# TxCorpi0x/concrete

Measured on AMD Instinct MI355X. Metric: PBS/sec (whole node) at N=1024 batch=4096; achieved HBM GB/s, higher is better.
Workload: dtype u64

## Files before the change

### concrete_amd/csrc/pbs.hip

```cpp
#include <type_traits>

#include "common.hpp"
#include "fft512.hpp"
#include "kernel_util.hpp"
#include "pbs.hpp"
#include "pbs1024_plan.hpp"
#include "pbs_hex.hpp"
#include "pbs_launch.hpp"

namespace chip {

static_assert(MAGIC_ALL_3 == RND_MAGIC_BITS + (RND_MAGIC_BITS << 22) + (RND_MAGIC_BITS << 43),
              "three limbs at shifts 0, 22, 43");

#ifndef FWD_LAST_VIA_WINDOW
#define FWD_LAST_VIA_WINDOW 1
#endif
#ifndef FWD_TW2_EARLY
#define FWD_TW2_EARLY 1
#endif
#ifndef DIAG_NOMAC
#define DIAG_NOMAC 0
#endif

#ifndef FWD_XBATCH
#define FWD_XBATCH 2
#endif
#ifndef PAIR_FLAGS
#define PAIR_FLAGS 1
#endif

#if defined(DIAG_NOXBAR)
constexpr bool XBAR = false;
#else
constexpr bool XBAR = true;
#endif
__device__ __forceinline__ void pair_signal(uint32_t* f, int h, uint32_t& cnt) {
  if constexpr (XBAR) group_signal<2>(f, h, cnt);
}
__device__ __forceinline__ void pair_wait(uint32_t* f, int h, uint32_t cnt, const SyncGuard& guard) {
  if constexpr (XBAR) group_wait<2>(f, h, cnt, guard);
}
__device__ __forceinline__ void xchg_barrier(uint32_t* f, int h, uint32_t& cnt, const SyncGuard& guard) {
  if constexpr (!XBAR) asm volatile("s_waitcnt lgkmcnt(0)" ::: "memory");
  else if constexpr (PAIR_FLAGS) group_sync<2>(f, h, cnt, guard);
  else pair_barrier();
}

template <int P, int L, bool RESID, bool STAMPS>
__global__ void __launch_bounds__(P * 128, 2)
pbs1024_pair_kernel(uint64_t* __restrict__ out, const uint64_t* __restrict__ out_idx,
                    const uint64_t* __restrict__ luts, const uint64_t* __restrict__ lut_idx,
                    const uint64_t* __restrict__ in, const uint64_t* __restrict__ in_idx,
                    const cplx* __restrict__ fbsk, uint32_t n, uint32_t base_log, uint32_t num_samples,
                    unsigned long long* __restrict__ resid_out, SyncGuard guard) {
  constexpr int K = 1, K1 = 2, N = 1024, LOG2_2N = 11, LIMBS = 3, RQ = K1 * L;
  constexpr int PER_I = K1 * LIMBS * RQ * 512;
  static_assert(XCH_SLOTS <= (int)PBS1024_XCH_SLOTS, "transpose scratch");
  static_assert(FFT512_TABLE_ENTRIES * sizeof(cplx) == PBS1024_TABLE_BYTES, "table bytes");
  constexpr int NW = 2 * P;
  constexpr int GROUP = L * 512;
  constexpr int NGRP = K1 * K1 * LIMBS;
  constexpr int GLDS = GROUP / 64 / NW;
  static_assert(GROUP % (64 * NW) == 0, "group split");

  extern __shared__ __attribute__((aligned(16))) char smem[];
  cplx* tbl = reinterpret_cast<cplx*>(smem);
  cplx* xch_all = tbl + FFT512_TABLE_ENTRIES;
  cplx* ring = xch_all + NW * PBS1024_XCH_SLOTS;
  uint32_t* pflags = reinterpret_cast<uint32_t*>(ring + 3 * GROUP);

  const int w = __builtin_amdgcn_readfirstlane(threadIdx.x >> 6);
  const int h = w & 1;
  uint32_t* pf = pflags + (w - h);
  const uint64_t hsign = (uint64_t)h << 63;
  const int lane = threadIdx.x & 63;
  const uint32_t s = blockIdx.x * P + (w >> 1);
  const bool active = s < num_samples;
  cplx* xch = xch_all + w * PBS1024_XCH_SLOTS;
  uint64_t* xch64 = reinterpret_cast<uint64_t*>(xch);
  cplx* mybox = xch;
  const cplx* partnerbox = xch_all + (w ^ 1) * PBS1024_XCH_SLOTS;
  cplx* partnermail = xch_all + (w ^ 1) * PBS1024_XCH_SLOTS;

  static_assert(NGRP % 3 == 0, "ring slot of a group must not depend on the step");
  const cplx* key_w = fbsk + (uint64_t)w * GLDS * 64;
  cplx* ring_w = ring + w * GLDS * 64;
  const uint32_t lane_b = (uint32_t)lane * (uint32_t)sizeof(cplx);
  auto issue_group = [&](const cplx* key_step, int r) __attribute__((always_inline)) {
    ring_issue<GLDS, true>(reinterpret_cast<const char*>(key_step + r * GROUP), ring_w + (r % 3) * GROUP, lane_b);
  };
  if (n > 0) {
    issue_group(key_w, 0);
    issue_group(key_w, 1);
  }

  build_fft512_tables(tbl, threadIdx.x, P * 128);
  if (lane == 0) pflags[w] = 0u;
  uint32_t pcnt = 0;
  __syncthreads();
  const Fft512Tables T = fft512_tables_at(tbl);

  const uint64_t* lwe = in + (active ? (in_idx ? in_idx[s] : s) : 0) * (uint64_t)(n + 1);
  const uint64_t* lut = luts + (active && lut_idx ? lut_idx[s] : 0ull) * (uint64_t)(K1 * N);

  uint64_t B[16];
  {
    const uint32_t bt = active ? modswitch(lwe[n], LOG2_2N) : 0u;
#pragma unroll
    for (int m = 0; m < 16; ++m) {
      const uint32_t src = (uint32_t)(lane + 64 * m + bt) & (2 * N - 1);
      const uint64_t v = active ? lut[h * N + (src & (N - 1))] : 0ull;
      B[m] = src < N ? 0ull - v : v;
    }
  }

  const int nrep = 64 - L * (int)base_log;
  const int logB = (int)base_log;
  const int32_t neg_base = -(1 << logB);
  const uint32_t half_m1 = (1u << (logB - 1)) - 1u;
  double max_resid = 0.0;
  uint64_t acc_t[NSTAMP] = {};
  uint64_t t_begin = 0, tp = 0;
  if constexpr (STAMPS) t_begin = stamp();

  cplx tw3[4];
  fwd_p3_tw(tw3, T, lane);

  uint64_t a_next = active ? lwe[0] : 0ull;
  for (uint32_t i = 0; i < n; ++i) {
    const cplx* key_step = key_w + (uint64_t)i * PER_I;
    const uint64_t ai = a_next;
    if (i + 1 < n) a_next = active ? lwe[i + 1] : 0ull;

    const uint32_t at = modswitch(ai, LOG2_2N);
    if constexpr (STAMPS) {
      tp = stamp();
      acc_t[7] += ai != 0ull && at != 0u;
    }

    uint32_t st[16];
    {
#pragma unroll
      for (int m = 0; m < 16; ++m) xch64[lane + 64 * m] = B[m];
      wave_lds_fence();
      const uint32_t o0 = ((uint32_t)(lane - (int)at) << 3) + 8u * N;
      const uint32_t khi = 1u << (nrep - 33);
      uint64_t rv[16];
#pragma unroll
      for (int m = 0; m < 16; ++m)
        rv[m] = *reinterpret_cast<const uint64_t*>(reinterpret_cast<const char*>(xch64) + ((o0 + 512u * m) & 8191u));
      __builtin_amdgcn_sched_barrier(0);
#pragma unroll
      for (int m = 0; m < 16; ++m) {
        const uint32_t o = o0 + 512u * m;
        const uint32_t s32 = (uint32_t)((int32_t)(o << 18) >> 31);
        const uint64_t rvs = rv[m] ^ (((uint64_t)s32 << 32) | s32);
        const uint64_t x = B[m] + rvs + (uint64_t)(s32 & 1u);
        st[m] = ((uint32_t)(x >> 32) + khi) >> (nrep - 32);
      }
      wave_lds_fence();
    }
    if constexpr (STAMPS) {
      uint64_t t = stamp();
      acc_t[0] += t - tp;
      tp = t;
    }

    cplx Xo[L][4], Xp[L][4];
    constexpr int XB = FWD_XBATCH;
#pragma unroll
    for (int q0 = 0; q0 < L; q0 += XB) {
      const int nq = (q0 + XB <= L) ? XB : L - q0;
      cplx out[XB][4];
      {
#pragma unroll
        for (int t = 0; t < XB; ++t) {
          if (t < nq) {
            cplx v[8];
            int32_t d[16];
#pragma unroll
            for (int m = 0; m < 16; ++m)
              d[m] = decomp_level32(st[m], (uint32_t)((q0 + t) * logB), logB, half_m1, neg_base, q0 + t + 1 < L);
#pragma unroll
            for (int m = 0; m < 8; ++m) v[m] = {(double)d[m], (double)d[m + 8]};
            cplx tw2[4];
            fwd_p2_tw(tw2, T, lane >> 3);
            if (FWD_TW2_EARLY) __builtin_amdgcn_sched_barrier(0);
            fft512_fwd_tw(v, xch, lane, tw2, tw3, hsign, [&]() __attribute__((always_inline)) {
              if (q0 > 0 && t == 0) pair_wait(pf, h, pcnt, guard);
            });
#pragma unroll
            for (int j = 0; j < 4; ++j) {
              Xo[q0 + t][j] = v[j];
              out[t][j] = v[4 + j];
            }
          }
        }
#pragma unroll
        for (int t = 0; t < XB; ++t)
          if (t < nq)
#pragma unroll
            for (int j = 0; j < 4; ++j) mybox[(t * 4 + j) * 64 + lane] = out[t][j];
      }
      const bool last_batch = q0 + XB >= L;
      if (!last_batch || !FWD_LAST_VIA_WINDOW) {
        xchg_barrier(pf, h, pcnt, guard);
#pragma unroll
        for (int t = 0; t < XB; ++t)
          if (t < nq)
#pragma unroll
            for (int j = 0; j < 4; ++j) Xp[q0 + t][j] = partnerbox[(t * 4 + j) * 64 + lane];
      }
#pragma unroll
      for (int t = 0; t < XB; ++t)
        if (t < nq)
#pragma unroll
          for (int j = 0; j < 4; ++j) pin(Xo[q0 + t][j]);
      if (q0 + XB < L) pair_signal(pf, h, pcnt);
    }
    if constexpr (STAMPS) {
      uint64_t t = stamp();
      acc_t[1] += t - tp;
      tp = t;
    }

    auto recombine = [&](const cplx (&v)[8], auto LIc) __attribute__((always_inline)) {
      constexpr int lr = decltype(LIc)::value;
#pragma unroll
      for (int m = 0; m < 8; ++m) {
        const double tr = RND_MAGIC - v[m].re, ti = RND_MAGIC - v[m].im;
        if constexpr (RESID) {
          max_resid = fmax(max_resid, fabs(v[m].re - (RND_MAGIC - tr)));
          max_resid = fmax(max_resid, fabs(v[m].im - (RND_MAGIC - ti)));
        }
        if constexpr (lr == 0) {
          B[m] += (uint64_t)__double_as_longlong(tr) - MAGIC_ALL_3;
          B[m + 8] += (uint64_t)__double_as_longlong(ti) - MAGIC_ALL_3;
        } else {
          B[m] += (uint64_t)__double_as_longlong(tr) << limb_shift(lr);
          B[m + 8] += (uint64_t)__double_as_longlong(ti) << limb_shift(lr);
        }
      }
    };
    static_for<0, LIMBS>([&](auto LI) __attribute__((always_inline)) {
      constexpr int li = decltype(LI)::value;
      cplx Ymine[4];
#pragma unroll
      for (int co = 0; co < K1; ++co) {
        cplx Y[4];
        if constexpr (DIAG_NOMAC) {
#pragma unroll
          for (int j = 0; j < 4; ++j) Y[j] = {0.0, 0.0};
        }
#pragma unroll
        for (int ro = 0; ro < K1; ++ro) {
          const int r = (li * K1 + co) * K1 + ro;
          const bool last_step = i + 1 >= n;
          if constexpr (STAMPS) {
            uint64_t t = stamp();
            acc_t[2] += t - tp;
            tp = t;
          }
          if (r + 1 < NGRP || !last_step) wait_vmcnt<GLDS>();
          else wait_vmcnt<0>();
          if constexpr (STAMPS) {
            uint64_t t = stamp();
            acc_t[8] += t - tp;
            tp = t;
          }
#ifndef DIAG_NOBAR
          pair_barrier();
#endif
          if constexpr (STAMPS) {
            uint64_t t = stamp();
            acc_t[5] += t - tp;
            tp = t;
          }
#ifndef DIAG_NODMA
          if (r + 2 < NGRP) issue_group(key_step, r + 2);
          else if (!last_step) issue_group(key_step + PER_I, r + 2 - NGRP);
#endif
          if constexpr (FWD_LAST_VIA_WINDOW && li == 0) {
            if (co == 0 && ro == 0) {
              constexpr int QL = (L - 1) / FWD_XBATCH * FWD_XBATCH;
#pragma unroll
              for (int q = QL; q < L; ++q)
#pragma unroll
                for (int j = 0; j < 4; ++j) Xp[q][j] = partnerbox[((q - QL) * 4 + j) * 64 + lane];
            }
          }
          const cplx* G = ring + (r % 3) * GROUP + (4 * h) * 64 + lane;
          cplx gv[L][4];
#pragma unroll
          for (int q = 0; q < L; ++q)
#pragma unroll
            for (int j = 0; j < 4; ++j) gv[q][j] = G[(q * 8 + j) * 64];
#pragma unroll
          for (int q = 0; q < (DIAG_NOMAC ? 0 : L); ++q) {
#pragma unroll
            for (int j = 0; j < 4; ++j) {
              const cplx x = ro == 0 ? Xo[q][j] : Xp[q][j];
              if (ro == 0 && q == 0) {
                Y[j].re = __builtin_fma(x.re, gv[q][j].re, -x.im * gv[q][j].im);
                Y[j].im = __builtin_fma(x.re, gv[q][j].im, x.im * gv[q][j].re);
              } else {
                Y[j].re = __builtin_fma(x.re, gv[q][j].re, __builtin_fma(-x.im, gv[q][j].im, Y[j].re));
                Y[j].im = __builtin_fma(x.re, gv[q][j].im, __builtin_fma(x.im, gv[q][j].re, Y[j].im));
              }
            }
          }
#pragma unroll
          for (int j = 0; j < 4; ++j) pin(Y[j]);
        }
        if (co == 0) {
#pragma unroll
          for (int j = 0; j < 4; ++j) Ymine[j] = Y[j];
        } else {
#pragma unroll
          for (int j = 0; j < 4; ++j) partnermail[j * 64 + lane] = Y[j];
        }
      }
      if constexpr (STAMPS) {
        uint64_t t = stamp();
        acc_t[2] += t - tp;
        tp = t;
      }
      xchg_barrier(pf, h, pcnt, guard);
      cplx vp[8];
#pragma unroll
      for (int j = 0; j < 4; ++j) {
        vp[j] = Ymine[j];
        vp[4 + j] = mybox[j * 64 + lane];
      }
      if constexpr (STAMPS) {
        uint64_t t = stamp();
        acc_t[3] += t - tp;
        tp = t;
      }
      cplx gi2[4];
      inv_p2_stage_tw(gi2, T, lane & 7);
      fft512_inv_tw(vp, xch, T, lane, gi2, hsign);
      recombine(vp, LI);
#pragma unroll
      for (int m = 0; m < 16; ++m) pin(B[m]);
      if constexpr (RESID) pin(max_resid);
      if constexpr (STAMPS) {
        uint64_t t = stamp();
        acc_t[4] += t - tp;
        tp = t;
      }
    });
  }

  if constexpr (STAMPS) {
    acc_t[6] = stamp() - t_begin;
    if (lane == 0 && resid_out) {
      unsigned long long* dst = resid_out + ((uint64_t)blockIdx.x * NW + w) * NSTAMP;
      for (int q = 0; q < NSTAMP; ++q) dst[q] = acc_t[q];
    }
  }

  uint64_t* o = out + (active ? (out_idx ? out_idx[s] : s) : 0) * (uint64_t)(K * N + 1);
  if (!active) {
  } else if (h == 0) {
#pragma unroll
    for (int m = 0; m < 16; ++m) xch64[lane + 64 * m] = B[m];
    wave_lds_fence();
#pragma unroll
    for (int m = 0; m < 16; ++m) {
      const int j = lane + 64 * m;
      const uint64_t v = xch64[(N - j) & (N - 1)];
      o[j] = j == 0 ? 0ull - v : v;
    }
  } else if (lane == 0) {
    o[K * N] = 0ull - B[0];
  }

  if constexpr (RESID && !STAMPS) report_resid(max_resid, lane, active, resid_out);
}

#ifndef SLOT_PF
#define SLOT_PF 6
#endif
#ifndef SLOT_FWD_PAIR
#define SLOT_FWD_PAIR 1
#endif
#ifndef SLOT_Y_EARLY
#define SLOT_Y_EARLY 1
#endif
#ifndef SLOT_QMAJOR
#define SLOT_QMAJOR 1
#endif
#ifndef SLOT_DEFAULT
#define SLOT_DEFAULT 1
#endif
constexpr int SLOT_MBOX = 512;
constexpr size_t pbs1024_pair_slot_lds_bytes() {
  return PBS1024_TABLE_BYTES + 2 * (size_t)PBS_PAIRS * (PBS1024_XCH_SLOTS + SLOT_MBOX) * 16 + 16;
}

__device__ __forceinline__ void slot_signal(uint32_t* ctr, int lane, uint32_t& cnt) {
  asm volatile("" ::: "memory");
  ++cnt;
  if (lane == 0) __hip_atomic_fetch_add(ctr, 1u, __ATOMIC_RELAXED, __HIP_MEMORY_SCOPE_WORKGROUP);
}

template <bool RESID, bool STAMPS>
__global__ void __launch_bounds__(PBS_PAIRS * 128, 2)
pbs1024_pair_slot_kernel(uint64_t* __restrict__ out, const uint64_t* __restrict__ out_idx,
                         const uint64_t* __restrict__ luts, const uint64_t* __restrict__ lut_idx,
                         const uint64_t* __restrict__ in, const uint64_t* __restrict__ in_idx,
                         const cplx* __restrict__ fbsk, uint32_t n, uint32_t base_log, uint32_t num_samples,
                         unsigned long long* __restrict__ resid_out, SyncGuard guard) {
  constexpr int K = 1, K1 = 2, N = 1024, LOG2_2N = 11, LIMBS = 3, L = 3, P = PBS_PAIRS, NW = 2 * P;
  constexpr int GROUP = L * 512;
  constexpr int PER_I = K1 * K1 * LIMBS * GROUP;
  constexpr int NKEY = LIMBS * K1 * K1 * L;
  constexpr int PF = SLOT_PF;
  constexpr int XS = (int)PBS1024_XCH_SLOTS, MB = SLOT_MBOX;
  static_assert(NW == 8, "one frequency slot per wave");
  static_assert(NKEY % PF == 0, "a key value's register must not depend on the step");
  static_assert(XCH_SLOTS <= XS, "transpose scratch");

  extern __shared__ __attribute__((aligned(16))) char smem[];
  cplx* tbl = reinterpret_cast<cplx*>(smem);
  cplx* xch_all = tbl + FFT512_TABLE_ENTRIES;
  cplx* mbox_all = xch_all + NW * XS;
  uint32_t* ctr = reinterpret_cast<uint32_t*>(mbox_all + NW * MB);

  const int w = __builtin_amdgcn_readfirstlane(threadIdx.x >> 6);
  const int h = w & 1;
  const int lane = threadIdx.x & 63;
  const uint32_t s = blockIdx.x * P + (w >> 1);
  const bool active = s < num_samples;
  cplx* xch = xch_all + w * XS;
  uint64_t* xch64 = reinterpret_cast<uint64_t*>(xch);
  cplx* mybox = mbox_all + w * MB + lane;
  cplx* slotbox = mbox_all + w * 64 + lane;

  const bool flip = w >= 4;
  const cplx* key_w = fbsk + (w * 64 + (flip ? 3 * GROUP : 0));
  const int gstride = flip ? -GROUP : GROUP;
  auto key_load = [&](const cplx* key_step, int t) __attribute__((always_inline)) {
    const int li = t / (K1 * K1 * L), co = t / (K1 * L) % K1, e = t % (K1 * L);
    const int ro = SLOT_QMAJOR ? e % K1 : e / L, q = SLOT_QMAJOR ? e / K1 : e % L, cr = co * K1 + ro;
    return (key_step + (li * K1 * K1 * GROUP + q * 512) + cr * gstride)[lane];
  };
  cplx g[PF] = {};
  if (n > 0) {
#pragma unroll
    for (int t = 0; t < PF; ++t) g[t] = key_load(key_w, t);
  }

  build_fft512_tables(tbl, threadIdx.x, P * 128);
  if (threadIdx.x == 0) *ctr = 0u;
  uint32_t rcnt = 0;
  __syncthreads();
  const Fft512Tables T = fft512_tables_at(tbl);

  const uint64_t* lwe = in + (active ? (in_idx ? in_idx[s] : s) : 0) * (uint64_t)(n + 1);
  const uint64_t* lut = luts + (active && lut_idx ? lut_idx[s] : 0ull) * (uint64_t)(K1 * N);

  uint64_t B[16];
  {
    const uint32_t bt = active ? modswitch(lwe[n], LOG2_2N) : 0u;
#pragma unroll
    for (int m = 0; m < 16; ++m) {
      const uint32_t src = (uint32_t)(lane + 64 * m + bt) & (2 * N - 1);
      const uint64_t v = active ? lut[h * N + (src & (N - 1))] : 0ull;
      B[m] = src < N ? 0ull - v : v;
    }
  }

  const int nrep = 64 - L * (int)base_log;
  const int logB = (int)base_log;
  const int32_t neg_base = -(1 << logB);
  const uint32_t half_m1 = (1u << (logB - 1)) - 1u;
  double max_resid = 0.0;
  uint64_t acc_t[NSTAMP] = {};
  uint64_t t_begin = 0, tp = 0;
  auto lap = [&](int k) __attribute__((always_inline)) {
    if constexpr (STAMPS) {
      const uint64_t t = stamp();
      acc_t[k] += t - tp;
      tp = t;
    }
  };
  if constexpr (STAMPS) t_begin = stamp();

  cplx tw3[4];
  fwd_p3_tw(tw3, T, lane);

  uint64_t a_next = active && n > 0 ? lwe[0] : 0ull;
  for (uint32_t i = 0; i < n; ++i) {
    const cplx* key_step = key_w + (uint64_t)i * PER_I;
    const cplx* key_next = i + 1 < n ? key_step + PER_I : key_step;
    const uint64_t ai = a_next;
    if (i + 1 < n) a_next = active ? lwe[i + 1] : 0ull;
    const uint32_t at = modswitch(ai, LOG2_2N);
    if constexpr (STAMPS) {
      tp = stamp();
      acc_t[7] += ai != 0ull && at != 0u;
    }

    uint32_t st[16];
    {
#pragma unroll
      for (int m = 0; m < 16; ++m) xch64[lane + 64 * m] = B[m];
      wave_lds_fence();
      const uint32_t o0 = ((uint32_t)(lane - (int)at) << 3) + 8u * N;
      const uint32_t khi = 1u << (nrep - 33);
      uint64_t rv[16];
#pragma unroll
      for (int m = 0; m < 16; ++m)
        rv[m] = *reinterpret_cast<const uint64_t*>(reinterpret_cast<const char*>(xch64) + ((o0 + 512u * m) & 8191u));
      __builtin_amdgcn_sched_barrier(0);
#pragma unroll
      for (int m = 0; m < 16; ++m) {
        const uint32_t o = o0 + 512u * m;
        const uint32_t s32 = (uint32_t)((int32_t)(o << 18) >> 31);
        const uint64_t rvs = rv[m] ^ (((uint64_t)s32 << 32) | s32);
        const uint64_t x = B[m] + rvs + (uint64_t)(s32 & 1u);
        st[m] = ((uint32_t)(x >> 32) + khi) >> (nrep - 32);
      }
      wave_lds_fence();
    }
    lap(0);

    cplx X[L][NW];
    cplx hold[8];
    (void)hold;
#pragma unroll
    for (int q = 0; q < L; ++q) {
      cplx v[8];
      int32_t d[16];
#pragma unroll
      for (int m = 0; m < 16; ++m)
        d[m] = decomp_level32(st[m], (uint32_t)(q * logB), logB, half_m1, neg_base, q + 1 < L);
#pragma unroll
      for (int m = 0; m < 8; ++m) v[m] = {(double)d[m], (double)d[m + 8]};
      cplx tw2[4];
      fwd_p2_tw(tw2, T, lane >> 3);
      if (FWD_TW2_EARLY) __builtin_amdgcn_sched_barrier(0);
#if SLOT_FWD_PAIR
      fft512_fwd_tw(v, xch, lane, tw2, tw3, 0ull, [&]() __attribute__((always_inline)) {
        if (q == 2) spin_until_ge(ctr, NW * rcnt, guard);
      });
      if (q == 0) {
#pragma unroll
        for (int k = 0; k < 8; ++k) hold[k] = v[k];
      } else {
#pragma unroll
        for (int k = 0; k < 8; ++k) {
          if (q == 1) mybox[k * 64] = hold[k], xch[k * 64 + lane] = v[k];
          else mybox[k * 64] = v[k];
        }
        lap(1);
        pair_barrier();
        lap(5);
#pragma unroll
        for (int u = 0; u < NW; ++u) {
          if (q == 1) X[0][u] = slotbox[u * MB], X[1][u] = xch_all[u * XS + w * 64 + lane];
          else X[2][u] = slotbox[u * MB];
        }
        slot_signal(ctr, lane, rcnt);
      }
#else
      fft512_fwd_tw(v, xch, lane, tw2, tw3, 0ull, []() __attribute__((always_inline)) {});
      if (q > 0) spin_until_ge(ctr, NW * rcnt, guard);
#pragma unroll
      for (int k = 0; k < 8; ++k) mybox[k * 64] = v[k];
      lap(1);
      pair_barrier();
      lap(5);
#pragma unroll
      for (int u = 0; u < NW; ++u) X[q][u] = slotbox[u * MB];
      slot_signal(ctr, lane, rcnt);
#endif
    }
    lap(1);

    auto recombine = [&](const cplx (&v)[8], auto LIc) __attribute__((always_inline)) {
      constexpr int lr = decltype(LIc)::value;
#pragma unroll
      for (int m = 0; m < 8; ++m) {
        const double tr = RND_MAGIC - v[m].re, ti = RND_MAGIC - v[m].im;
        if constexpr (RESID) {
          max_resid = fmax(max_resid, fabs(v[m].re - (RND_MAGIC - tr)));
          max_resid = fmax(max_resid, fabs(v[m].im - (RND_MAGIC - ti)));
        }
        if constexpr (lr == 0) {
          B[m] += (uint64_t)__double_as_longlong(tr) - MAGIC_ALL_3;
          B[m + 8] += (uint64_t)__double_as_longlong(ti) - MAGIC_ALL_3;
        } else {
          B[m] += (uint64_t)__double_as_longlong(tr) << limb_shift(lr);
          B[m + 8] += (uint64_t)__double_as_longlong(ti) << limb_shift(lr);
        }
      }
    };
    auto window = [&](auto LIc, auto COc) __attribute__((always_inline)) {
      constexpr int li = decltype(LIc)::value, co = decltype(COc)::value;
      cplx Y[P];
#pragma unroll
      for (int e = 0; e < K1 * L; ++e) {
        const int ro = SLOT_QMAJOR ? e % K1 : e / L, q = SLOT_QMAJOR ? e / K1 : e % L;
        const int t = (li * K1 + co) * K1 * L + e;
        const cplx gv = g[t % PF];
#pragma unroll
        for (int c = 0; c < P; ++c) {
          const cplx x = X[q][2 * c + ro];
          if (e == 0) {
            Y[c].re = __builtin_fma(x.re, gv.re, -x.im * gv.im);
            Y[c].im = __builtin_fma(x.re, gv.im, x.im * gv.re);
          } else {
            Y[c].re = __builtin_fma(x.re, gv.re, __builtin_fma(-x.im, gv.im, Y[c].re));
            Y[c].im = __builtin_fma(x.re, gv.im, __builtin_fma(x.im, gv.re, Y[c].im));
          }
        }
        g[t % PF] = t + PF < NKEY ? key_load(key_step, t + PF) : key_load(key_next, t + PF - NKEY);
      }
#pragma unroll
      for (int c = 0; c < P; ++c) pin(Y[c]);
      if (co == 0) spin_until_ge(ctr, NW * rcnt, guard);
#pragma unroll
      for (int c = 0; c < P; ++c) mbox_all[(2 * c + co) * MB + w * 64 + lane] = Y[c];
    };
    if (SLOT_Y_EARLY) window(std::integral_constant<int, 0>{}, std::integral_constant<int, 0>{});
    static_for<0, LIMBS>([&](auto LI) __attribute__((always_inline)) {
      constexpr int li = decltype(LI)::value;
      if (!SLOT_Y_EARLY) window(LI, std::integral_constant<int, 0>{});
      window(LI, std::integral_constant<int, 1>{});
      lap(2);
      pair_barrier();
      lap(5);
      cplx vp[8];
#pragma unroll
      for (int k = 0; k < 8; ++k) vp[k] = mybox[k * 64];
      slot_signal(ctr, lane, rcnt);
      lap(3);
      if constexpr (SLOT_Y_EARLY && li + 1 < LIMBS) {
        window(std::integral_constant<int, li + 1>{}, std::integral_constant<int, 0>{});
        lap(2);
      }
      cplx gi2[4];
      inv_p2_stage_tw(gi2, T, lane & 7);
      fft512_inv_tw(vp, xch, T, lane, gi2, 0ull);
      recombine(vp, LI);
#pragma unroll
      for (int m = 0; m < 16; ++m) pin(B[m]);
      if constexpr (RESID) pin(max_resid);
      lap(4);
    });
  }

  if constexpr (STAMPS) {
    acc_t[6] = stamp() - t_begin;
    if (lane == 0 && resid_out) {
      unsigned long long* dst = resid_out + ((uint64_t)blockIdx.x * NW + w) * NSTAMP;
      for (int q = 0; q < NSTAMP; ++q) dst[q] = acc_t[q];
    }
  }

  uint64_t* o = out + (active ? (out_idx ? out_idx[s] : s) : 0) * (uint64_t)(K * N + 1);
  if (!active) {
  } else if (h == 0) {
#pragma unroll
    for (int m = 0; m < 16; ++m) xch64[lane + 64 * m] = B[m];
    wave_lds_fence();
#pragma unroll
    for (int m = 0; m < 16; ++m) {
      const int j = lane + 64 * m;
      const uint64_t v = xch64[(N - j) & (N - 1)];
      o[j] = j == 0 ? 0ull - v : v;
    }
  } else if (lane == 0) {
    o[K * N] = 0ull - B[0];
  }

  if constexpr (RESID && !STAMPS) report_resid(max_resid, lane, active, resid_out);
}

template <bool RESID, bool STAMPS>
static int launch_slot_t(const PbsArgs& a) {
  constexpr int P = PBS_PAIRS;
  const size_t lds = pbs1024_pair_slot_lds_bytes();
  static_assert(pbs1024_pair_slot_lds_bytes() <= 160 * 1024, "LDS of one CU");
  if (!pbs1024_exact(1, 3, a.base_log)) {
    set_error("pbs: N=1024 l=3 logB=%u is outside the exact range", a.base_log);
    return -2;
  }
  return launch_fused(pbs1024_pair_slot_kernel<RESID, STAMPS>, P, P * 128, lds, a);
}

static int launch_slot(const PbsArgs& a) {
  static const bool stamps = getenv("CONCRETE_HIP_PBS_STAMPS") && atoi(getenv("CONCRETE_HIP_PBS_STAMPS"));
  if (stamps) return launch_slot_t<true, true>(a);
  return a.resid ? launch_slot_t<true, false>(a) : launch_slot_t<false, false>(a);
}

template <int P, int L, bool RESID, bool STAMPS>
static int launch_pair_t(const PbsArgs& a) {
  const size_t lds = pbs1024_pair_lds_bytes(L, P);
  if (!pbs1024_exact(1, L, a.base_log)) {
    set_error("pbs: N=1024 l=%d logB=%u is outside the exact range", L, a.base_log);
    return -2;
  }
  return launch_fused(pbs1024_pair_kernel<P, L, RESID, STAMPS>, P, P * 128, lds, a);
}

static uint32_t device_cus() {
  static uint32_t cus[64] = {};
  int dev = 0;
  CHIP_CHECK(hipGetDevice(&dev));
  if (dev < 0 || dev >= 64) return 256;
  if (!cus[dev]) {
    int n = 0;
    CHIP_CHECK(hipDeviceGetAttribute(&n, hipDeviceAttributeMultiprocessorCount, dev));
    cus[dev] = n > 0 ? (uint32_t)n : 256u;
  }
  return cus[dev];
}

template <int P, int L>
static int launch_pair_p(const PbsArgs& a) {
  static const bool stamps = getenv("CONCRETE_HIP_PBS_STAMPS") && atoi(getenv("CONCRETE_HIP_PBS_STAMPS"));
  if (stamps) return launch_pair_t<P, L, true, true>(a);
  return a.resid ? launch_pair_t<P, L, true, false>(a) : launch_pair_t<P, L, false, false>(a);
}

static PbsArgs pbs_args_range(const PbsArgs& a, uint32_t start, uint32_t count) {
  PbsArgs r = a;
  r.num_samples = count;
  if (a.in_idx) r.in_idx = a.in_idx + start;
  else r.in = a.in + (uint64_t)start * (a.n + 1);
  if (a.out_idx) r.out_idx = a.out_idx + start;
  else r.out = a.out + (uint64_t)start * (a.k * a.N + 1);
  if (a.lut_idx) r.lut_idx = a.lut_idx + start;
  return r;
}

template <int L>
static int launch_pair(const PbsArgs& a) {
  if (a.num_samples == 0) return 0;
  const char* fe = getenv("CONCRETE_HIP_PBS_PAIRS");
  const int forced = fe ? atoi(fe) : 0;
  const uint32_t cus = device_cus();
  const int P = forced == 1 || forced == 2 || forced == 4 ? forced
                : a.num_samples <= cus ? 1 : a.num_samples <= 2 * cus ? 2 : 4;
  if (L == 3) {
    const char* se = getenv("CONCRETE_HIP_PBS_SLOT");
    const int sl = se ? atoi(se) : -1;
    if (sl == 1) return launch_slot(a);
    const char* he = getenv("CONCRETE_HIP_PBS_HEX");
    const int hx = he ? atoi(he) : -1;
    if (hx == 1 || hx == 2) return pbs1024_hex_launch(a, hx);
    if (hx != 0 && !fe && !getenv("CONCRETE_HIP_PBS_QUAD") && !getenv("CONCRETE_HIP_PBS_STAMPS")) {
      const Pbs1024Plan plan = plan_pbs1024(a.num_samples, cus);
      uint32_t start = 0;
      int rc = 0;
      if (plan.pair) {
        const PbsArgs part = pbs_args_range(a, start, plan.pair);
        rc = (sl == 0 || !SLOT_DEFAULT) ? launch_pair_p<4, L>(part) : launch_slot(part);
        start += plan.pair;
      }
      if (rc == 0 && plan.hex2) {
        rc = pbs1024_hex_launch(pbs_args_range(a, start, plan.hex2), 2);
        start += plan.hex2;
      }
      if (rc == 0 && plan.hex1) rc = pbs1024_hex_launch(pbs_args_range(a, start, plan.hex1), 1);
      return rc;
    }
  }
  if (L == 3 && P <= 2 && !getenv("CONCRETE_HIP_PBS_STAMPS")) {
    const char* qe = getenv("CONCRETE_HIP_PBS_QUAD");
    const int q = qe ? atoi(qe) : -1;
    if (q == 1 || q == 2) return pbs1024_quad_launch(a, q);
    if (q != 0 && P == 1) return pbs1024_quad_launch(a, 1);
  }
  if (P == 1) return launch_pair_p<1, L>(a);
  if (P == 2) return launch_pair_p<2, L>(a);
  return launch_pair_p<4, L>(a);
}

int pbs_launch(const PbsArgs& a) {
  const KeyKind kind = key_format(a.k, a.N, a.level).kind;
  if (kind == KeyKind::GENERIC) return pbs_generic_launch(a);
  if (kind == KeyKind::N2048) return pbs2048_launch(a);
  if (kind == KeyKind::K2N1024) return pbs1024k2_launch(a);
  if (kind == KeyKind::SMALL) return pbs_small_launch(a);
  if (kind == KeyKind::N1024 && a.limbs == 3) {
    switch (a.level) {
      case 1: return launch_pair<1>(a);
      case 2: return launch_pair<2>(a);
      case 3: return launch_pair<3>(a);
      default: break;
    }
  }
  set_error("unsupported PBS parameters: N=%u k=%u level=%u limbs=%u", a.N, a.k, a.level, a.limbs);
  return -2;
}

}
```

Baseline: 106,900.

## Overlap first window with level-2 forward FFT and fold inverse twiddle into rounding

Splits the first product window so its level-0/1 products are computed inside the level-2 forward FFT, after the LDS exchange and before the last twiddle stage, to hide LDS latency. Inlines the inverse FFT stages and folds the final per-output twiddle multiply into the rounding step, using tangent factoring and an FMA against the magic constant. Also recomputes the lane id at the end to ease register pressure, and adds optional interleaved-forward and split-inverse paths that are off by default. This risks extra register pressure and relies on the ordering static_asserts holding.

```diff
diff --git a/concrete_amd/csrc/pbs.hip b/concrete_amd/csrc/pbs.hip
--- a/concrete_amd/csrc/pbs.hip
+++ b/concrete_amd/csrc/pbs.hip
@@ -395,6 +395,37 @@
 #ifndef SLOT_DEFAULT
 #define SLOT_DEFAULT 1
 #endif
+#ifndef SLOT_INV_FOLD
+#define SLOT_INV_FOLD 1
+#endif
+#ifndef SLOT_FWD_IL
+#define SLOT_FWD_IL 0
+#endif
+#ifndef SLOT_L2_WINDOW
+#define SLOT_L2_WINDOW 1
+#endif
+#ifndef SLOT_INV_SPLIT
+#define SLOT_INV_SPLIT 0
+#endif
+#ifndef SLOT_LANE_AGAIN
+#define SLOT_LANE_AGAIN (SLOT_L2_WINDOW && !SLOT_INV_FOLD ? 2 : 1)
+#endif
+static_assert(!SLOT_FWD_IL || SLOT_FWD_PAIR, "the interleaved pair is traded in one exchange");
+static_assert(!SLOT_L2_WINDOW || (SLOT_Y_EARLY && SLOT_QMAJOR && SLOT_FWD_PAIR),
+              "the first window's first four products must need levels 0 and 1 only");
+static_assert(!SLOT_INV_SPLIT || SLOT_Y_EARLY, "the split window is the early one");
+__device__ __forceinline__ double psi_tan(int m) {
+  constexpr double TAN[8] = {0.0,
+                             0x1.975f5e0553158p-3,
+                             0x1.a827999fcef32p-2,
+                             0x1.561b82ab7f990p-1,
+                             1.0,
+                             0x1.7f218e25a7461p+0,
+                             0x1.3504f333f9de6p+1,
+                             0x1.41bfee2424771p+2};
+  return TAN[m];
+}
+__device__ __forceinline__ void slot_order() { __builtin_amdgcn_sched_barrier(0); }
 constexpr int SLOT_MBOX = 512;
 constexpr size_t pbs1024_pair_slot_lds_bytes() {
   return PBS1024_TABLE_BYTES + 2 * (size_t)PBS_PAIRS * (PBS1024_XCH_SLOTS + SLOT_MBOX) * 16 + 16;
@@ -529,81 +560,11 @@
     lap(0);
 
     cplx X[L][NW];
-    cplx hold[8];
-    (void)hold;
-#pragma unroll
-    for (int q = 0; q < L; ++q) {
-      cplx v[8];
-      int32_t d[16];
-#pragma unroll
-      for (int m = 0; m < 16; ++m)
-        d[m] = decomp_level32(st[m], (uint32_t)(q * logB), logB, half_m1, neg_base, q + 1 < L);
-#pragma unroll
-      for (int m = 0; m < 8; ++m) v[m] = {(double)d[m], (double)d[m + 8]};
-      cplx tw2[4];
-      fwd_p2_tw(tw2, T, lane >> 3);
-      if (FWD_TW2_EARLY) __builtin_amdgcn_sched_barrier(0);
-#if SLOT_FWD_PAIR
-      fft512_fwd_tw(v, xch, lane, tw2, tw3, 0ull, [&]() __attribute__((always_inline)) {
-        if (q == 2) spin_until_ge(ctr, NW * rcnt, guard);
-      });
-      if (q == 0) {
-#pragma unroll
-        for (int k = 0; k < 8; ++k) hold[k] = v[k];
-      } else {
-#pragma unroll
-        for (int k = 0; k < 8; ++k) {
-          if (q == 1) mybox[k * 64] = hold[k], xch[k * 64 + lane] = v[k];
-          else mybox[k * 64] = v[k];
-        }
-        lap(1);
-        pair_barrier();
-        lap(5);
-#pragma unroll
-        for (int u = 0; u < NW; ++u) {
-          if (q == 1) X[0][u] = slotbox[u * MB], X[1][u] = xch_all[u * XS + w * 64 + lane];
-          else X[2][u] = slotbox[u * MB];
-        }
-        slot_signal(ctr, lane, rcnt);
-      }
-#else
-      fft512_fwd_tw(v, xch, lane, tw2, tw3, 0ull, []() __attribute__((always_inline)) {});
-      if (q > 0) spin_until_ge(ctr, NW * rcnt, guard);
-#pragma unroll
-      for (int k = 0; k < 8; ++k) mybox[k * 64] = v[k];
-      lap(1);
-      pair_barrier();
-      lap(5);
-#pragma unroll
-      for (int u = 0; u < NW; ++u) X[q][u] = slotbox[u * MB];
-      slot_signal(ctr, lane, rcnt);
-#endif
-    }
-    lap(1);
-
-    auto recombine = [&](const cplx (&v)[8], auto LIc) __attribute__((always_inline)) {
-      constexpr int lr = decltype(LIc)::value;
-#pragma unroll
-      for (int m = 0; m < 8; ++m) {
-        const double tr = RND_MAGIC - v[m].re, ti = RND_MAGIC - v[m].im;
-        if constexpr (RESID) {
-          max_resid = fmax(max_resid, fabs(v[m].re - (RND_MAGIC - tr)));
-          max_resid = fmax(max_resid, fabs(v[m].im - (RND_MAGIC - ti)));
-        }
-        if constexpr (lr == 0) {
-          B[m] += (uint64_t)__double_as_longlong(tr) - MAGIC_ALL_3;
-          B[m + 8] += (uint64_t)__double_as_longlong(ti) - MAGIC_ALL_3;
-        } else {
-          B[m] += (uint64_t)__double_as_longlong(tr) << limb_shift(lr);
-          B[m + 8] += (uint64_t)__double_as_longlong(ti) << limb_shift(lr);
-        }
-      }
-    };
-    auto window = [&](auto LIc, auto COc) __attribute__((always_inline)) {
+    const int hi = lane >> 3, lo = lane & 7;
+    auto window_part = [&](cplx (&Y)[P], auto LIc, auto COc, auto E0c, auto E1c) __attribute__((always_inline)) {
       constexpr int li = decltype(LIc)::value, co = decltype(COc)::value;
-      cplx Y[P];
-#pragma unroll
-      for (int e = 0; e < K1 * L; ++e) {
+#pragma unroll
+      for (int e = decltype(E0c)::value; e < decltype(E1c)::value; ++e) {
         const int ro = SLOT_QMAJOR ? e % K1 : e / L, q = SLOT_QMAJOR ? e / K1 : e % L;
         const int t = (li * K1 + co) * K1 * L + e;
         const cplx gv = g[t % PF];
@@ -620,17 +581,183 @@
         }
         g[t % PF] = t + PF < NKEY ? key_load(key_step, t + PF) : key_load(key_next, t + PF - NKEY);
       }
+    };
+    auto window_send = [&](cplx (&Y)[P], auto COc) __attribute__((always_inline)) {
+      constexpr int co = decltype(COc)::value;
 #pragma unroll
       for (int c = 0; c < P; ++c) pin(Y[c]);
       if (co == 0) spin_until_ge(ctr, NW * rcnt, guard);
 #pragma unroll
       for (int c = 0; c < P; ++c) mbox_all[(2 * c + co) * MB + w * 64 + lane] = Y[c];
     };
-    if (SLOT_Y_EARLY) window(std::integral_constant<int, 0>{}, std::integral_constant<int, 0>{});
+    constexpr std::integral_constant<int, 0> I0{};
+    constexpr std::integral_constant<int, K1 * L> IE{};
+    constexpr std::integral_constant<int, 2 * K1> IQ2{};
+    constexpr std::integral_constant<int, K1 * L / 2> IH{};
+    auto window = [&](auto LIc, auto COc) __attribute__((always_inline)) {
+      cplx Y[P];
+      window_part(Y, LIc, COc, I0, IE);
+      window_send(Y, COc);
+    };
+    auto digits = [&](cplx (&v)[8], int q) __attribute__((always_inline)) {
+      int32_t d[16];
+#pragma unroll
+      for (int m = 0; m < 16; ++m)
+        d[m] = decomp_level32(st[m], (uint32_t)(q * logB), logB, half_m1, neg_base, q + 1 < L);
+#pragma unroll
+      for (int m = 0; m < 8; ++m) v[m] = {(double)d[m], (double)d[m + 8]};
+    };
+    cplx Y0[P];
+    (void)Y0;
+#if SLOT_FWD_IL
+    {
+      cplx v0[8], v1[8];
+      digits(v0, 0);
+      digits(v1, 1);
+      cplx tw2[4];
+      fwd_p2_tw(tw2, T, hi);
+      if (FWD_TW2_EARLY) __builtin_amdgcn_sched_barrier(0);
+      fwd_p1(v0);
+      fwd_p1(v1);
+      xpose_hi(v0);
+      xpose_hi(v1);
+      geo8<false>(v0, tw2);
+      fwd_w2(v0, xch, hi, lo);
+      wave_lds_fence();
+      slot_order();
+      geo8<false>(v1, tw2);
+      slot_order();
+      fwd_r2(v0, xch, hi, lo);
+      wave_lds_fence();
+      fwd_w2(v1, xch, hi, lo);
+      wave_lds_fence();
+      slot_order();
+      geo8<false>(v0, tw3);
+      slot_order();
+      fwd_r2(v1, xch, hi, lo);
+      wave_lds_fence();
+      geo8<false>(v1, tw3);
+#pragma unroll
+      for (int k = 0; k < 8; ++k) mybox[k * 64] = v0[k], xch[k * 64 + lane] = v1[k];
+      lap(1);
+      pair_barrier();
+      lap(5);
+#pragma unroll
+      for (int u = 0; u < NW; ++u) X[0][u] = slotbox[u * MB], X[1][u] = xch_all[u * XS + w * 64 + lane];
+      slot_signal(ctr, lane, rcnt);
+    }
+#endif
+    cplx hold[8];
+    (void)hold;
+#pragma unroll
+    for (int q = SLOT_FWD_IL ? 2 : 0; q < L; ++q) {
+      cplx v[8];
+      digits(v, q);
+      cplx tw2[4];
+      fwd_p2_tw(tw2, T, hi);
+      if (FWD_TW2_EARLY) __builtin_amdgcn_sched_barrier(0);
+#if SLOT_FWD_PAIR
+      if (SLOT_L2_WINDOW && q == 2) {
+        fwd_p1(v);
+        xpose_hi(v);
+        geo8<false>(v, tw2);
+        spin_until_ge(ctr, NW * rcnt, guard);
+        fwd_w2(v, xch, hi, lo);
+        wave_lds_fence();
+        fwd_r2(v, xch, hi, lo);
+        wave_lds_fence();
+        slot_order();
+        window_part(Y0, I0, I0, I0, IQ2);
+        slot_order();
+        geo8<false>(v, tw3);
+      } else {
+        fft512_fwd_tw(v, xch, lane, tw2, tw3, 0ull, [&]() __attribute__((always_inline)) {
+          if (q == 2) spin_until_ge(ctr, NW * rcnt, guard);
+        });
+      }
+      if (q == 0) {
+#pragma unroll
+        for (int k = 0; k < 8; ++k) hold[k] = v[k];
+      } else {
+#pragma unroll
+        for (int k = 0; k < 8; ++k) {
+          if (q == 1) mybox[k * 64] = hold[k], xch[k * 64 + lane] = v[k];
+          else mybox[k * 64] = v[k];
+        }
+        lap(1);
+        pair_barrier();
+        lap(5);
+#pragma unroll
+        for (int u = 0; u < NW; ++u) {
+          if (q == 1) X[0][u] = slotbox[u * MB], X[1][u] = xch_all[u * XS + w * 64 + lane];
+          else X[2][u] = slotbox[u * MB];
+        }
+        slot_signal(ctr, lane, rcnt);
+      }
+#else
+      fft512_fwd_tw(v, xch, lane, tw2, tw3, 0ull, []() __attribute__((always_inline)) {});
+      if (q > 0) spin_until_ge(ctr, NW * rcnt, guard);
+#pragma unroll
+      for (int k = 0; k < 8; ++k) mybox[k * 64] = v[k];
+      lap(1);
+      pair_barrier();
+      lap(5);
+#pragma unroll
+      for (int u = 0; u < NW; ++u) X[q][u] = slotbox[u * MB];
+      slot_signal(ctr, lane, rcnt);
+#endif
+    }
+    lap(1);
+
+    auto recombine = [&](const cplx (&v)[8], auto LIc) __attribute__((always_inline)) {
+      constexpr int lr = decltype(LIc)::value;
+      double rnd = RND_MAGIC;
+      if (SLOT_INV_FOLD) pin(rnd);
+#pragma unroll
+      for (int m = 0; m < 8; ++m) {
+        double tr, ti;
+        if (SLOT_INV_FOLD && m > 0) {
+          const bool cot = m > 4;
+          const double c = psi_pow(cot ? 8 - m : m).re, t = psi_tan(cot ? 8 - m : m);
+          const double ur = cot ? __builtin_fma(t, v[m].re, v[m].im) : __builtin_fma(t, v[m].im, v[m].re);
+          const double ui = cot ? __builtin_fma(t, v[m].im, -v[m].re) : __builtin_fma(-t, v[m].re, v[m].im);
+          if constexpr (RESID) {
+            double pr = c * ur, pi = c * ui;
+            pin(pr), pin(pi);
+            tr = RND_MAGIC - pr, ti = RND_MAGIC - pi;
+            max_resid = fmax(max_resid, fabs(pr - (RND_MAGIC - tr)));
+            max_resid = fmax(max_resid, fabs(pi - (RND_MAGIC - ti)));
+          } else {
+            tr = __builtin_fma(-c, ur, rnd), ti = __builtin_fma(-c, ui, rnd);
+          }
+        } else {
+          tr = RND_MAGIC - v[m].re, ti = RND_MAGIC - v[m].im;
+          if constexpr (RESID) {
+            max_resid = fmax(max_resid, fabs(v[m].re - (RND_MAGIC - tr)));
+            max_resid = fmax(max_resid, fabs(v[m].im - (RND_MAGIC - ti)));
+          }
+        }
+        if constexpr (lr == 0) {
+          B[m] += (uint64_t)__double_as_longlong(tr) - MAGIC_ALL_3;
+          B[m + 8] += (uint64_t)__double_as_longlong(ti) - MAGIC_ALL_3;
+        } else {
+          B[m] += (uint64_t)__double_as_longlong(tr) << limb_shift(lr);
+          B[m + 8] += (uint64_t)__double_as_longlong(ti) << limb_shift(lr);
+        }
+      }
+    };
+    if (SLOT_L2_WINDOW) {
+      window_part(Y0, I0, I0, IQ2, IE);
+      window_send(Y0, I0);
+    } else if (SLOT_Y_EARLY) {
+      window(I0, I0);
+    }
     static_for<0, LIMBS>([&](auto LI) __attribute__((always_inline)) {
       constexpr int li = decltype(LI)::value;
-      if (!SLOT_Y_EARLY) window(LI, std::integral_constant<int, 0>{});
-      window(LI, std::integral_constant<int, 1>{});
+      constexpr std::integral_constant<int, 1> I1{};
+      constexpr std::integral_constant<int, li + 1> LN{};
+      if (!SLOT_Y_EARLY) window(LI, I0);
+      window(LI, I1);
       lap(2);
       pair_barrier();
       lap(5);
@@ -639,13 +766,45 @@
       for (int k = 0; k < 8; ++k) vp[k] = mybox[k * 64];
       slot_signal(ctr, lane, rcnt);
       lap(3);
-      if constexpr (SLOT_Y_EARLY && li + 1 < LIMBS) {
-        window(std::integral_constant<int, li + 1>{}, std::integral_constant<int, 0>{});
+      cplx gi2[4];
+      if constexpr (SLOT_INV_SPLIT && li + 1 < LIMBS) {
+        cplx Yn[P];
+        window_part(Yn, LN, I0, I0, IH);
+        slot_order();
+        inv_p1(vp, 0ull);
+        inv_w1(vp, xch, hi, lo);
+        wave_lds_fence();
+        slot_order();
+        window_part(Yn, LN, I0, IH, IE);
+        window_send(Yn, I0);
         lap(2);
-      }
-      cplx gi2[4];
-      inv_p2_stage_tw(gi2, T, lane & 7);
-      fft512_inv_tw(vp, xch, T, lane, gi2, 0ull);
+        slot_order();
+        inv_p2_stage_tw(gi2, T, lo);
+        inv_r1(vp, xch, hi, lo);
+        wave_lds_fence();
+      } else {
+        if constexpr (SLOT_Y_EARLY && li + 1 < LIMBS) {
+          window(LN, I0);
+          lap(2);
+        }
+        inv_p2_stage_tw(gi2, T, lo);
+        inv_p1(vp, 0ull);
+        inv_w1(vp, xch, hi, lo);
+        wave_lds_fence();
+        inv_r1(vp, xch, hi, lo);
+        wave_lds_fence();
+      }
+      {
+        cplx t1[8];
+#pragma unroll
+        for (int t = 0; t < 8; ++t) t1[t] = T.T1[hi * T1_STRIDE + 8 * t + lo];
+        geo8<true, true>(vp, gi2);
+#pragma unroll
+        for (int t = 0; t < 8; ++t) vp[t] = cmulc(vp[t], t1[t]);
+        xpose_hi(vp);
+        if (SLOT_INV_FOLD) dft8<true>(vp);
+        else inv_p3(vp);
+      }
       recombine(vp, LI);
 #pragma unroll
       for (int m = 0; m < 16; ++m) pin(B[m]);
@@ -662,6 +821,9 @@
     }
   }
 
+  const int lane_x = SLOT_LANE_AGAIN == 2 || (SLOT_LANE_AGAIN == 1 && RESID)
+                         ? (int)__builtin_amdgcn_mbcnt_hi(~0u, __builtin_amdgcn_mbcnt_lo(~0u, 0u))
+                         : lane;
   uint64_t* o = out + (active ? (out_idx ? out_idx[s] : s) : 0) * (uint64_t)(K * N + 1);
   if (!active) {
   } else if (h == 0) {
@@ -670,15 +832,15 @@
     wave_lds_fence();
 #pragma unroll
     for (int m = 0; m < 16; ++m) {
-      const int j = lane + 64 * m;
+      const int j = lane_x + 64 * m;
       const uint64_t v = xch64[(N - j) & (N - 1)];
       o[j] = j == 0 ? 0ull - v : v;
     }
-  } else if (lane == 0) {
+  } else if (lane_x == 0) {
     o[K * N] = 0ull - B[0];
   }
 
-  if constexpr (RESID && !STAMPS) report_resid(max_resid, lane, active, resid_out);
+  if constexpr (RESID && !STAMPS) report_resid(max_resid, lane_x, active, resid_out);
 }
 
 template <bool RESID, bool STAMPS>
```

Result: faster. 108,900 (median of 6 runs) (+1.9%).
